# LightwheelAI/street-gaussians-ns

Measured on NVIDIA H100. Metric: rendered frames/sec (fwd+bwd) at 1920x1280, 1M+32x10k Gaussians, higher is better.
Workload: dtype f32

## Files before the change

include/sgn_raster.h:

```cpp
#ifndef SGN_RASTER_H_
#define SGN_RASTER_H_

#include <stddef.h>
#include <stdint.h>

#ifdef __cplusplus
extern "C" {
#endif

#define SGN_ABI_VERSION 2
#define SGN_MAX_FOURIER 8
#define SGN_RECORD_FLOATS 12

typedef enum sgn_status {
    SGN_OK = 0,
    SGN_ERR_INVALID = -1,
    SGN_ERR_CUDA = -2,
    SGN_ERR_WORKSPACE = -3,
    SGN_ERR_OVERFLOW = -4
} sgn_status;


typedef struct sgn_segment {
    int32_t row0;
// ... 53 lines not shown
#define SGN_TUNE_ACC_NO_ROW_SKIP 16
#define SGN_TUNE_FWD_TMA 32

const char* sgn_last_error(void);
int sgn_abi_version(void);
long long sgn_launch_count(void);
size_t sgn_sizeof_segment(void);
size_t sgn_sizeof_segment_grads(void);
size_t sgn_sizeof_camera(void);

int sgn_upload(const void* host, size_t bytes, void* dev, void* stream);

int sgn_project_fwd(const sgn_segment* segs_dev, int nseg, int N, int num_chunks, const sgn_camera* cam,
                    float* records, int32_t* radii, int32_t* num_tiles_hit, uint16_t* tile_bbox,
                    int32_t* tiles_touched, uint32_t* touch_mask, void* stream);

int sgn_project_bwd(const sgn_segment* segs_dev, const sgn_segment_grads* grads_dev, int nseg, int N, int num_chunks,
                    const sgn_camera* cam, const float* records, const int32_t* radii,
                    const float* v_records, void* stream);
int sgn_project_bwd_range(const sgn_segment* segs_dev, const sgn_segment_grads* grads_dev, int nseg, int N, int num_chunks,
                          const sgn_camera* cam, const float* records, const int32_t* radii, const float* v_records,
                          int chunk_begin, int chunk_end, void* stream);

int sgn_l1_project_fwd(int N, const float* means, const float* scales, float glob_scale, const float* quats,
                       const sgn_camera* cam, float* xys, float* depths, int32_t* radii, float* conics,
                       float* compensation, int32_t* num_tiles_hit, float* cov3d, void* stream);
int sgn_l1_project_bwd(int N, const float* means, const float* scales, float glob_scale, const float* quats,
                       const sgn_camera* cam, const int32_t* radii, const float* v_xys, const float* v_depths,
                       const float* v_conics, float* v_means, float* v_scales, float* v_quats, void* stream);
int sgn_l1_sh(int N, int K, int degree, const float* viewdirs, const float* coeffs, const float* v_colors,
              float* colors, float* v_coeffs, void* stream);

int sgn_bin_count(int N, const sgn_camera* cam, const float* records, const int32_t* radii,
                  const uint16_t* tile_bbox, int32_t* tiles_touched, uint32_t* touch_mask, void* stream);
size_t sgn_bin_scan_scratch_bytes(int N);
int sgn_bin_scan(int N, const float* records, const int32_t* radii, const int32_t* tiles_touched,
                 int32_t* order, int32_t* cum, int64_t* total_dev, void* scratch, size_t scratch_bytes, void* stream);
size_t sgn_bin_sort_scratch_bytes(int64_t M);
int sgn_bin_sort(int N, int64_t M, const sgn_camera* cam, const float* records, const int32_t* radii,
                 const uint16_t* tile_bbox, const uint32_t* touch_mask, const int32_t* order, const int32_t* cum,
                 int32_t* sorted_ids , int32_t* tile_bins , void* scratch, size_t scratch_bytes,
                 void* stream);
int sgn_bin_sort_capped(int N, int64_t capacity, const int64_t* total_dev, int32_t* overflow_dev, const sgn_camera* cam,
                        const float* records, const int32_t* radii, const uint16_t* tile_bbox, const uint32_t* touch_mask,
                        const int32_t* order, const int32_t* cum, int32_t* sorted_ids, int32_t* tile_bins, void* scratch,
                        size_t scratch_bytes, void* stream);
int sgn_bin_local_cap(void);
size_t sgn_bin_local_scratch_bytes(int64_t M, int tiles);
int sgn_bin_local_count(int N, const sgn_camera* cam, const float* records, const int32_t* radii, const uint16_t* tile_bbox,
                        const uint32_t* touch_mask, int32_t* tile_count, int32_t* tile_start, int64_t* info_dev, void* scratch,
                        size_t scratch_bytes, void* stream);
int sgn_bin_local_sort(int N, int64_t M, int longest_list, const sgn_camera* cam, const float* records, const int32_t* radii,
// ... 145 lines not shown
```

street-gaussians-ns_b200/_lib.py:

```python
from __future__ import annotations

import ctypes as C
import os

HERE = os.path.dirname(os.path.abspath(__file__))
LIB_PATH = os.path.join(HERE, "libsgn_raster.so")
MAX_FOURIER = 8
RECORD_FLOATS = 12


class SgnError(RuntimeError):
    pass


class Segment(C.Structure):
    _fields_ = [
        ("row0", C.c_int32), ("count", C.c_int32), ("F", C.c_int32), ("cls", C.c_int32),
        ("has_pose", C.c_int32), ("chunk0", C.c_int32),
        ("R", C.c_float * 9), ("t", C.c_float * 3), ("q", C.c_float * 4), ("idft", C.c_float * MAX_FOURIER),
        ("means", C.c_void_p), ("scales", C.c_void_p), ("quats", C.c_void_p),
        ("features_dc", C.c_void_p), ("features_rest", C.c_void_p), ("opacities", C.c_void_p),
    ]


# ... 88 lines not shown
    ]


_lib = None

EXPORTS = [
    "sgn_last_error", "sgn_abi_version", "sgn_launch_count", "sgn_sizeof_segment", "sgn_sizeof_segment_grads", "sgn_sizeof_camera",
    "sgn_upload", "sgn_bin_count", "sgn_project_fwd", "sgn_project_bwd", "sgn_l1_project_fwd", "sgn_l1_project_bwd", "sgn_l1_sh", "sgn_bin_scan_scratch_bytes", "sgn_bin_scan",
    "sgn_bin_sort_scratch_bytes", "sgn_bin_sort", "sgn_bin_class_scratch_bytes", "sgn_bin_class_lists", "sgn_blend_sched_ints",
    "sgn_blend_fwd", "sgn_blend_bwd", "sgn_sizeof_adam_tensor", "sgn_adam_chunk_elems", "sgn_adam_step",
    "sgn_loss_scratch_bytes", "sgn_loss_fwd", "sgn_loss_bwd", "sgn_ssim_workspace_bytes", "sgn_ssim_fwd", "sgn_ssim_bwd",
    "sgn_sizeof_densify_segment", "sgn_densify_stats",
    "sgn_sizeof_refine_config", "sgn_sizeof_refine_tensors", "sgn_refine_decide", "sgn_refine_apply",
    "sgn_bin_local_cap", "sgn_bin_local_scratch_bytes", "sgn_bin_local_count", "sgn_bin_local_sort",
    "sgn_project_bwd_range", "sgn_allreduce_sym", "sgn_blend_extra_fwd", "sgn_blend_extra_bwd",
    "sgn_bin_sort_capped", "sgn_visible_flags", "sgn_visible_union",
]
AR_MAX_SLICES = 48


def load():
    global _lib
    if _lib is not None:
        return _lib
    path = os.environ.get("SGN_RASTER_LIB", LIB_PATH)
    if not os.path.exists(path):
        raise SgnError(
            f"{path} is missing. Build it with `python street-gaussians-ns_b200/build.py` "
            "(or __graft_entry__.build()). There is no CPU fallback for the rasterizer.")
    L = C.CDLL(path)
    vp, i32, i64, sz = C.c_void_p, C.c_int, C.c_int64, C.c_size_t
    L.sgn_last_error.restype = C.c_char_p
    L.sgn_abi_version.restype = C.c_int
    L.sgn_launch_count.restype = C.c_longlong
    for f in ("sgn_sizeof_segment", "sgn_sizeof_segment_grads", "sgn_sizeof_camera"):
        getattr(L, f).restype = sz
    L.sgn_upload.argtypes = [vp, sz, vp, vp]
    L.sgn_project_fwd.argtypes = [vp, i32, i32, i32, C.POINTER(CameraStruct), vp, vp, vp, vp, vp, vp, vp]
    L.sgn_project_bwd.argtypes = [vp, vp, i32, i32, i32, C.POINTER(CameraStruct), vp, vp, vp, vp]
    L.sgn_project_bwd_range.argtypes = [vp, vp, i32, i32, i32, C.POINTER(CameraStruct), vp, vp, vp, i32, i32, vp]
    L.sgn_project_bwd_range.restype = C.c_int
    L.sgn_allreduce_sym.argtypes = [vp, vp, vp, i32, i32, i32, C.POINTER(C.c_int64), C.POINTER(C.c_int64), C.POINTER(C.c_int32),
                                    C.POINTER(C.c_int64), C.POINTER(C.c_int64), vp, C.c_float, i32, vp]
    L.sgn_visible_flags.argtypes = [vp, i64, vp, vp]
    L.sgn_visible_union.argtypes = [vp, i64, i32, i64, vp, vp]
    L.sgn_allreduce_sym.restype = L.sgn_visible_flags.restype = L.sgn_visible_union.restype = C.c_int
    L.sgn_blend_extra_fwd.argtypes = [C.POINTER(CameraStruct), C.POINTER(BlendOpts), vp, vp, vp, vp, vp, vp, i32, vp, vp]
    L.sgn_blend_extra_bwd.argtypes = [C.POINTER(CameraStruct), C.POINTER(BlendOpts), vp, vp, vp, vp, vp, vp, i32, vp, vp, vp, vp]
    L.sgn_blend_extra_fwd.restype = L.sgn_blend_extra_bwd.restype = C.c_int
    fl = C.c_float
    L.sgn_l1_project_fwd.argtypes = [i32, vp, vp, fl, vp, C.POINTER(CameraStruct), vp, vp, vp, vp, vp, vp, vp, vp]
    L.sgn_l1_project_bwd.argtypes = [i32, vp, vp, fl, vp, C.POINTER(CameraStruct), vp, vp, vp, vp, vp, vp, vp, vp]
    L.sgn_l1_sh.argtypes = [i32, i32, i32, vp, vp, vp, vp, vp, vp]
    for f in ("sgn_l1_project_fwd", "sgn_l1_project_bwd", "sgn_l1_sh"):
        getattr(L, f).restype = C.c_int
    L.sgn_bin_scan_scratch_bytes.argtypes = [i32]
    L.sgn_bin_scan_scratch_bytes.restype = sz
    L.sgn_bin_scan.argtypes = [i32, vp, vp, vp, vp, vp, vp, vp, sz, vp]
    L.sgn_bin_count.argtypes = [i32, C.POINTER(CameraStruct), vp, vp, vp, vp, vp, vp]
    L.sgn_bin_count.restype = C.c_int
    L.sgn_bin_sort_scratch_bytes.argtypes = [i64]
    L.sgn_bin_sort_scratch_bytes.restype = sz
    L.sgn_bin_sort.argtypes = [i32, i64, C.POINTER(CameraStruct), vp, vp, vp, vp, vp, vp, vp, vp, vp, sz, vp]
    L.sgn_bin_sort_capped.argtypes = [i32, i64, vp, vp, C.POINTER(CameraStruct), vp, vp, vp, vp, vp, vp, vp, vp, vp, sz, vp]
    L.sgn_bin_sort_capped.restype = C.c_int
    L.sgn_bin_local_cap.restype = C.c_int
    L.sgn_bin_local_scratch_bytes.argtypes = [i64, i32]
    L.sgn_bin_local_scratch_bytes.restype = sz
    L.sgn_bin_local_count.argtypes = [i32, C.POINTER(CameraStruct), vp, vp, vp, vp, vp, vp, vp, vp, sz, vp]
    L.sgn_bin_local_count.restype = C.c_int
    L.sgn_bin_local_sort.argtypes = [i32, i64, i32, C.POINTER(CameraStruct), vp, vp, vp, vp, vp, vp, vp, vp, vp, vp, vp, sz, vp]
    L.sgn_bin_local_sort.restype = C.c_int
    L.sgn_bin_class_scratch_bytes.argtypes = [i32]
# ... 49 lines not shown
```

street-gaussians-ns_b200/csrc/binning.cu:

```cuda
#include <cub/cub.cuh>

#include "sgn_touch.cuh"

static inline size_t align_up(size_t x, size_t a) { return (x + a - 1) / a * a; }

__global__ void __launch_bounds__(256)
count_tiles_kernel(int N, int width, int height, int bw, const float4* __restrict__ records, const int32_t* __restrict__ radii,
                   const ushort4* __restrict__ tile_bbox, int32_t* __restrict__ tiles_touched, uint32_t* __restrict__ touch_mask) {
    const int g = blockIdx.x * blockDim.x + threadIdx.x;
    const bool vis = (g < N) && radii[g] > 0;
    ushort4 bb = make_ushort4(0, 0, 0, 0);
    TouchCtx t = {};
    if (vis) {
        bb = tile_bbox[g];
        t = make_touch_ctx(records[3 * (size_t)g], records[3 * (size_t)g + 1]);
    }
    uint32_t mask;
    const int n = count_touched_tiles(vis, t, bb, width, height, bw, mask);
    if (g < N) { tiles_touched[g] = n; touch_mask[g] = mask; }
}

extern "C" int sgn_bin_count(int N, const sgn_camera* cam, const float* records, const int32_t* radii,
                             const uint16_t* tile_bbox, int32_t* tiles_touched, uint32_t* touch_mask, void* stream) {
    SGN_RANGE("sgn_bin_count");
// ... 20 lines not shown
    }
    keys[g] = key;
    vals[g] = payload;
}

struct PermutedCount {
    const int32_t* order;
    const int32_t* counts;
    __host__ __device__ int32_t operator()(int i) const { return counts[order[i] & 0x7fffffff]; }
};

__global__ void write_total_kernel(const int32_t* __restrict__ cum, int N, int64_t* __restrict__ total) {
    if (threadIdx.x == 0 && blockIdx.x == 0) *total = (N > 0) ? (int64_t)cum[N - 1] : 0;
}

struct ScanLayout {
    size_t keys_in, keys_out, vals_in, temp, temp_bytes, total;
};
static ScanLayout scan_layout(int N) {
    ScanLayout L;
    const size_t n = (size_t)(N > 0 ? N : 1);
    size_t t1 = 0, t2 = 0;
    cub::DeviceRadixSort::SortPairs(nullptr, t1, (const uint32_t*)nullptr, (uint32_t*)nullptr, (const int32_t*)nullptr,
                                    (int32_t*)nullptr, (int)n, 0, 32);
    cub::DeviceScan::InclusiveSum(nullptr, t2, (const int32_t*)nullptr, (int32_t*)nullptr, (int)n);
    L.keys_in = 0;
    L.keys_out = align_up(n * 4, 256);
    L.vals_in = L.keys_out + align_up(n * 4, 256);
    L.temp = L.vals_in + align_up(n * 4, 256);
    L.temp_bytes = t1 > t2 ? t1 : t2;
    L.total = L.temp + align_up(L.temp_bytes, 256) + 256;
    return L;
}

extern "C" size_t sgn_bin_scan_scratch_bytes(int N) { return scan_layout(N).total; }

extern "C" int sgn_bin_scan(int N, const float* records, const int32_t* radii, const int32_t* tiles_touched,
                            int32_t* order , int32_t* cum,
                            int64_t* total_dev, void* scratch, size_t scratch_bytes, void* stream_) {
    SGN_RANGE("sgn_bin_scan");
    cudaStream_t stream = (cudaStream_t)stream_;
    SGN_REQUIRE(records && radii && tiles_touched && order && cum && total_dev && scratch, "sgn_bin_scan: null pointer");
    const ScanLayout L = scan_layout(N);
    if (scratch_bytes < L.total) {
// ... 6 lines not shown
        uint32_t* keys_out = (uint32_t*)(base + L.keys_out);
        int32_t* vals_in = (int32_t*)(base + L.vals_in);
        depth_keys_kernel<<<(N + 255) / 256, 256, 0, stream>>>(N, reinterpret_cast<const float4*>(records), radii, keys_in, vals_in);
        SGN_CHECK_LAUNCH("depth_keys_kernel");
        size_t temp = L.temp_bytes;
        SGN_CHECK_CUDA(cub::DeviceRadixSort::SortPairs(base + L.temp, temp, keys_in, keys_out, vals_in, order, N, 0, 32, stream));
        sgn_count_launch(1);
        cub::CountingInputIterator<int> idx(0);
        cub::TransformInputIterator<int32_t, PermutedCount, cub::CountingInputIterator<int>> it(idx, PermutedCount{order, tiles_touched});
        temp = L.temp_bytes;
        SGN_CHECK_CUDA(cub::DeviceScan::InclusiveSum(base + L.temp, temp, it, cum, N, stream));
        sgn_count_launch(1);
    }
    write_total_kernel<<<1, 32, 0, stream>>>(cum, N, total_dev);
    SGN_CHECK_LAUNCH("write_total_kernel");
    return SGN_OK;
}

#define HUGE_AREA 1024

__device__ __forceinline__ int nth_set_bit(uint32_t m, int k) {
    int pos = 0;
#pragma unroll
    for (int w = 16; w > 0; w >>= 1) {
        const int c = __popc(m & ((1u << w) - 1u));
        if (k >= c) { k -= c; m >>= w; pos += w; }
    }
    return pos;
}

// ... 141 lines not shown
        for (int b = 0; b < r.ar && r.pos < end; b += 32) {
            const int ti = b + lane;
            const int tx = r.x0 + ti % r.wd, ty = r.y0 + ti / r.wd;
            const bool ok = (ti < r.ar) && tile_touched(r.c, tx, ty, width, height, bw);
            const unsigned bal = __ballot_sync(0xffffffffu, ok);
            const int my = r.pos + __popc(bal & lt);
            if (ok && my < end) {
                keys[my] = (uint16_t)(ty * tiles_x + tx);
                vals[my] = r.pl;
            }
            r.pos += __popc(bal);
        }
    }
}

__global__ void __launch_bounds__(256)
bin_edges_kernel(int64_t M, const uint16_t* __restrict__ keys_sorted, int32_t* __restrict__ tile_bins) {
    const int64_t i = (int64_t)blockIdx.x * blockDim.x + threadIdx.x;
    if (i >= M) return;
    const int32_t cur = (int32_t)keys_sorted[i];
    if (i == 0) tile_bins[2 * cur] = 0;
    else {
        const int32_t prev = (int32_t)keys_sorted[i - 1];
        if (prev != cur) {
            tile_bins[2 * prev + 1] = (int32_t)i;
            tile_bins[2 * cur] = (int32_t)i;
        }
    }
    if (i == M - 1) tile_bins[2 * cur + 1] = (int32_t)M;
}

__global__ void __launch_bounds__(256)
bin_edges_capped_kernel(int64_t cap, const int64_t* __restrict__ total, const uint16_t* __restrict__ keys_sorted, int32_t* __restrict__ tile_bins,
                        int32_t* __restrict__ overflow) {
    const int64_t i = (int64_t)blockIdx.x * blockDim.x + threadIdx.x;
    const int64_t M = min(*total, cap);
    if (i == 0 && *total > cap) *overflow = 1;
    if (i >= M) return;
    const int32_t cur = (int32_t)keys_sorted[i];
    if (i == 0) tile_bins[2 * cur] = 0;
    else {
        const int32_t prev = (int32_t)keys_sorted[i - 1];
        if (prev != cur) {
            tile_bins[2 * prev + 1] = (int32_t)i;
            tile_bins[2 * cur] = (int32_t)i;
        }
    }
    if (i == M - 1) tile_bins[2 * cur + 1] = (int32_t)M;
}

struct SortLayout {
    size_t keys_in, keys_out, vals_in, big, temp, temp_bytes, total;
};

static SortLayout sort_layout(int64_t M) {
    SortLayout L;
    const size_t m = (size_t)(M > 0 ? M : 1);
    size_t temp = 0;
    cub::DeviceRadixSort::SortPairs(nullptr, temp, (const uint16_t*)nullptr, (uint16_t*)nullptr, (const int32_t*)nullptr,
                                    (int32_t*)nullptr, (int64_t)m, 0, 16);
    L.keys_in = 0;
    L.keys_out = align_up(L.keys_in + m * 2, 256);
    L.vals_in = align_up(L.keys_out + m * 2, 256);
// ... 38 lines not shown
    SGN_REQUIRE(!total_dev || tile_bits <= 16, "sgn_bin_sort_capped: %d tiles leave no 16-bit key for the padding", tiles);
    emit_keys_kernel<<<(N + 255) / 256, 256, 0, stream>>>(N, tiles_x, reinterpret_cast<const ushort4*>(tile_bbox), touch_mask, order, cum, (int)M,
                                                          total_dev, (uint16_t)((1u << tile_bits) - 1u), keys_in, vals_in, big_ranks,
                                                          big_count);
    SGN_CHECK_LAUNCH("emit_keys_kernel");
    int sms = 0, dev = 0;
    SGN_CHECK_CUDA(cudaGetDevice(&dev));
    SGN_CHECK_CUDA(cudaDeviceGetAttribute(&sms, cudaDevAttrMultiProcessorCount, dev));
    emit_big_kernel<<<4 * sms, EMIT_BIG_THREADS, 0, stream>>>(tiles_x, cam->width, cam->height, bw, reinterpret_cast<const float4*>(records),
                                                 reinterpret_cast<const ushort4*>(tile_bbox), order, cum, (int)M, big_ranks, big_count,
                                                 keys_in, vals_in);
    SGN_CHECK_LAUNCH("emit_big_kernel");
    size_t temp = L.temp_bytes;
    SGN_CHECK_CUDA(cub::DeviceRadixSort::SortPairs(base + L.temp, temp, keys_in, keys_out, vals_in, sorted_ids, M, 0, tile_bits, stream));
    sgn_count_launch(1);
    if (total_dev) {
        bin_edges_capped_kernel<<<(unsigned)((M + 255) / 256), 256, 0, stream>>>(M, total_dev, keys_out, tile_bins, overflow_dev);
        SGN_CHECK_LAUNCH("bin_edges_capped_kernel");
    } else {
        bin_edges_kernel<<<(unsigned)((M + 255) / 256), 256, 0, stream>>>(M, keys_out, tile_bins);
        SGN_CHECK_LAUNCH("bin_edges_kernel");
    }
    return SGN_OK;
}

extern "C" int sgn_bin_sort(int N, int64_t M, const sgn_camera* cam, const float* records, const int32_t* radii,
                            const uint16_t* tile_bbox, const uint32_t* touch_mask, const int32_t* order, const int32_t* cum,
                            int32_t* sorted_ids, int32_t* tile_bins, void* scratch, size_t scratch_bytes, void* stream_) {
    SGN_RANGE("sgn_bin_sort");
    return bin_sort_impl(N, M, nullptr, nullptr, cam, records, radii, tile_bbox, touch_mask, order, cum, sorted_ids, tile_bins, scratch,
                         scratch_bytes, stream_);
}

extern "C" int sgn_bin_sort_capped(int N, int64_t capacity, const int64_t* total_dev, int32_t* overflow_dev, const sgn_camera* cam,
                                   const float* records, const int32_t* radii, const uint16_t* tile_bbox, const uint32_t* touch_mask,
// ... 121 lines not shown
```

street-gaussians-ns_b200/csrc/project.cu:

```cuda
#include <stdarg.h>
#include <stdlib.h>
#include <string.h>

#include "sgn_exact.cuh"
#include "sgn_touch.cuh"

static thread_local char g_err[512] = "";
void sgn_set_error(const char* fmt, ...) {
    va_list ap;
    va_start(ap, fmt);
    vsnprintf(g_err, sizeof(g_err), fmt, ap);
    va_end(ap);
}
#include <atomic>
static std::atomic<long long> g_launches{0};
void sgn_count_launch(int n) { g_launches.fetch_add(n, std::memory_order_relaxed); }
extern "C" long long sgn_launch_count(void) { return g_launches.load(std::memory_order_relaxed); }
extern "C" const char* sgn_last_error(void) { return g_err; }
extern "C" int sgn_abi_version(void) { return SGN_ABI_VERSION; }
extern "C" size_t sgn_sizeof_segment(void) { return sizeof(sgn_segment); }
extern "C" size_t sgn_sizeof_segment_grads(void) { return sizeof(sgn_segment_grads); }
extern "C" size_t sgn_sizeof_camera(void) { return sizeof(sgn_camera); }

extern "C" int sgn_upload(const void* host, size_t bytes, void* dev, void* stream) {
// ... 29 lines not shown
        for (int i = threadIdx.x; i < n; i += blockDim.x) dst[i] = __ldg(src + i);
    }
}
__device__ __forceinline__ void coop_store(float* __restrict__ dst, const float* __restrict__ src, int n) {
    if ((reinterpret_cast<uintptr_t>(dst) & 15u) == 0) {
        const int n4 = n >> 2;
        const float4* s4 = reinterpret_cast<const float4*>(src);
        float4* d4 = reinterpret_cast<float4*>(dst);
        for (int i = threadIdx.x; i < n4; i += blockDim.x) d4[i] = s4[i];
        for (int i = (n4 << 2) + threadIdx.x; i < n; i += blockDim.x) dst[i] = src[i];
    } else {
        for (int i = threadIdx.x; i < n; i += blockDim.x) dst[i] = src[i];
    }
}

__global__ void __launch_bounds__(CH)
project_fwd_direct_kernel(const sgn_segment* __restrict__ segs, int nseg, const sgn_camera cam,
                   float4* __restrict__ records, int32_t* __restrict__ radii, int32_t* __restrict__ num_tiles_hit,
                   ushort4* __restrict__ tile_bbox, int32_t* __restrict__ tiles_touched, uint32_t* __restrict__ touch_mask) {
    extern __shared__ int s_chunk0[];
    for (int i = threadIdx.x; i < nseg; i += blockDim.x) s_chunk0[i] = segs[i].chunk0;
    __syncthreads();
    const int si = find_segment_by_chunk(s_chunk0, nseg, blockIdx.x);
    const sgn_segment& sg = segs[si];
    const int i = (blockIdx.x - sg.chunk0) * CH + threadIdx.x;
    const bool active = i < sg.count;
    const size_t g = (size_t)sg.row0 + i;
    const int K = (cam.sh_degree + 1) * (cam.sh_degree + 1);
    bool vis = false;
    ushort4 bb = make_ushort4(0, 0, 0, 0);
    TouchCtx tc = {};
    if (active) {

    float m[3], ls[3], q[4];
#pragma unroll
    for (int k = 0; k < 3; ++k) { m[k] = __ldg(sg.means + 3 * (size_t)i + k); ls[k] = __ldg(sg.scales + 3 * (size_t)i + k); }
    {
        const float4 qq = __ldg(reinterpret_cast<const float4*>(sg.quats) + i);
        q[0] = qq.x; q[1] = qq.y; q[2] = qq.z; q[3] = qq.w;
    }
    SgnProj st;
    vis = sgn_project_exact(sg, cam, m, ls, q, st);

    float rgb[3] = {0.f, 0.f, 0.f};
    float opac = 0.f;
    int aux = 0;
    if (vis) {
        float c0[3] = {0.f, 0.f, 0.f};
        for (int f = 0; f < sg.F; ++f) {
            const float w = sg.idft[f];
#pragma unroll
            for (int ch = 0; ch < 3; ++ch) c0[ch] += __ldg(sg.features_dc + ((size_t)i * sg.F + f) * 3 + ch) * w;
        }
        if (cam.sh_degree > 0) {
            float d[3] = {st.mw[0] - cam.cam_pos[0], st.mw[1] - cam.cam_pos[1], st.mw[2] - cam.cam_pos[2]};
            const float n = sqrtf(d[0] * d[0] + d[1] * d[1] + d[2] * d[2]);
            d[0] /= n; d[1] /= n; d[2] /= n;
// ... 28 lines not shown
    radii[g] = st.radius;
    num_tiles_hit[g] = vis ? (st.tmax[0] - st.tmin[0]) * (st.tmax[1] - st.tmin[1]) : 0;
    bb = make_ushort4((unsigned short)st.tmin[0], (unsigned short)st.tmin[1],
                      (unsigned short)st.tmax[0], (unsigned short)st.tmax[1]);
    tile_bbox[g] = bb;
    if (vis) tc = make_touch_ctx(make_float4(st.xy[0], st.xy[1], st.conic[0], st.conic[1]), make_float4(st.conic[2], opac, 0.f, 0.f));
    }
    uint32_t mask;
    const int nt = count_touched_tiles(vis, tc, bb, cam.width, cam.height, cam.block_width, mask);
    if (active) {
        tiles_touched[g] = nt;
        touch_mask[g] = mask;
    }
}

__global__ void __launch_bounds__(CH)
project_fwd_staged_kernel(const sgn_segment* __restrict__ segs, int nseg, const sgn_camera cam,
                   float4* __restrict__ records, int32_t* __restrict__ radii, int32_t* __restrict__ num_tiles_hit,
                   ushort4* __restrict__ tile_bbox, int32_t* __restrict__ tiles_touched, uint32_t* __restrict__ touch_mask) {
    extern __shared__ int s_chunk0[];
    __shared__ __align__(16) float s_rest[CH * MAX_REST];
    __shared__ __align__(16) float s_dc[CH * MAX_DC];
    __shared__ __align__(16) float s_means[CH * 3];
    __shared__ __align__(16) float s_scales[CH * 3];
    __shared__ float s_geo[CH][9];
    __shared__ int s_row[CH];
    __shared__ int s_warp_base[CH / 32 + 1];
    for (int i = threadIdx.x; i < nseg; i += blockDim.x) s_chunk0[i] = segs[i].chunk0;
    __syncthreads();
    const int si = find_segment_by_chunk(s_chunk0, nseg, blockIdx.x);
    const sgn_segment& sg = segs[si];
    const int r0 = (blockIdx.x - sg.chunk0) * CH;
    const int rows = min(CH, sg.count - r0);
    const int tid = threadIdx.x, lane = tid & 31, warp = tid >> 5;
// ... 2 lines not shown
    coop_load(s_means, sg.means + 3 * (size_t)r0, rows * 3);
    coop_load(s_scales, sg.scales + 3 * (size_t)r0, rows * 3);
    __syncthreads();

    const bool active = tid < rows;
    const size_t g = (size_t)sg.row0 + r0 + tid;
    const int cls_bit = sg.cls == 1 ? SGN_AUX_OBJECT : 0;
    bool vis = false;
    SgnProj st;
    if (active) {
        const float m[3] = {s_means[3 * tid], s_means[3 * tid + 1], s_means[3 * tid + 2]};
        const float ls[3] = {s_scales[3 * tid], s_scales[3 * tid + 1], s_scales[3 * tid + 2]};
        const float4 qq = __ldg(reinterpret_cast<const float4*>(sg.quats) + r0 + tid);
        const float q[4] = {qq.x, qq.y, qq.z, qq.w};
        vis = sgn_project_exact(sg, cam, m, ls, q, st);
        radii[g] = st.radius;
        num_tiles_hit[g] = vis ? (st.tmax[0] - st.tmin[0]) * (st.tmax[1] - st.tmin[1]) : 0;
        tile_bbox[g] = make_ushort4((unsigned short)st.tmin[0], (unsigned short)st.tmin[1],
                                    (unsigned short)st.tmax[0], (unsigned short)st.tmax[1]);
        float4* rec = records + 3 * g;
        rec[0] = make_float4(st.xy[0], st.xy[1], st.conic[0], st.conic[1]);
        if (!vis) {
            rec[1] = make_float4(st.conic[2], 0.f, 0.f, 0.f);
            rec[2] = make_float4(0.f, 0.f, __int_as_float(cls_bit), 0.f);
            tiles_touched[g] = 0;
            touch_mask[g] = 0u;
        }
    }
    const unsigned bal = __ballot_sync(0xffffffffu, vis);
    if (lane == 0) s_warp_base[warp + 1] = __popc(bal);
// ... 88 lines not shown
        float4* rec = records + 3 * gb;
        rec[1] = make_float4(ge[4], opac, rgb[0], rgb[1]);
        rec[2] = make_float4(rgb[2], ge[5], __int_as_float(aux), 0.f);
        bb = tile_bbox[gb];
        tc = make_touch_ctx(make_float4(ge[0], ge[1], ge[2], ge[3]), make_float4(ge[4], opac, 0.f, 0.f));
    }
    if ((warp << 5) >= nvis) return;
    uint32_t mask;
    const int nt = count_touched_tiles(mine, tc, bb, cam.width, cam.height, cam.block_width, mask);
    if (mine) {
        tiles_touched[gb] = nt;
        touch_mask[gb] = mask;
    }
}

extern "C" int sgn_project_fwd(const sgn_segment* segs_dev, int nseg, int N, int num_chunks, const sgn_camera* cam,
                               float* records, int32_t* radii, int32_t* num_tiles_hit, uint16_t* tile_bbox,
                               int32_t* tiles_touched, uint32_t* touch_mask, void* stream) {
    SGN_RANGE("sgn_project_fwd");
    SGN_REQUIRE(segs_dev && cam && records && radii && num_tiles_hit && tile_bbox && tiles_touched && touch_mask,
                "sgn_project_fwd: null pointer");
    SGN_REQUIRE(nseg >= 1 && nseg <= SGN_MAX_SEGMENTS, "sgn_project_fwd: nseg=%d out of range [1,%d]", nseg, SGN_MAX_SEGMENTS);
    SGN_REQUIRE(N >= 0 && num_chunks >= 0, "sgn_project_fwd: negative size");
    SGN_REQUIRE(cam->block_width >= 2 && cam->block_width <= 16, "block_width must be between 2 and 16 (got %d)", cam->block_width);
    SGN_REQUIRE(cam->sh_degree >= 0 && cam->sh_degree <= 3 && cam->sh_degree_to_use >= 0 && cam->sh_degree_to_use <= cam->sh_degree,
                "sh_degree must be in [0,3] and sh_degree_to_use <= sh_degree");
    SGN_REQUIRE((cam->width + cam->block_width - 1) / cam->block_width < 65536 && (cam->height + cam->block_width - 1) / cam->block_width < 65536,
                "image too large for 16-bit tile coordinates");
    SGN_REQUIRE(sgn_aligned16(records), "records must be 16-byte aligned");
    if (N == 0 || num_chunks == 0) return SGN_OK;
    const char* staged_env = getenv("SGN_PROJECT_STAGED");
    if (staged_env && staged_env[0] == '1')
        project_fwd_staged_kernel<<<num_chunks, CH, nseg * sizeof(int), (cudaStream_t)stream>>>(
            segs_dev, nseg, *cam, reinterpret_cast<float4*>(records), radii, num_tiles_hit,
            reinterpret_cast<ushort4*>(tile_bbox), tiles_touched, touch_mask);
    else
        project_fwd_direct_kernel<<<num_chunks, CH, nseg * sizeof(int), (cudaStream_t)stream>>>(
            segs_dev, nseg, *cam, reinterpret_cast<float4*>(records), radii, num_tiles_hit,
            reinterpret_cast<ushort4*>(tile_bbox), tiles_touched, touch_mask);
    SGN_CHECK_LAUNCH("project_fwd_kernel");
    return SGN_OK;
}

__device__ __forceinline__ void sgn_project_vjp(const sgn_camera& cam, const SgnProj& st, const float v_xy[2], float v_depth,
                                                const float v_conic[3], float vmw[3], float vs[3], float vqr[4]) {
    const float* W = cam.viewmat;
    const float fx = cam.fx, fy = cam.fy;
    float vpv[3];
    {
        const float rw = 1.f / (st.pv[2] + 1e-6f);
        const float vx = fx * v_xy[0], vy = fy * v_xy[1];
        vpv[0] = vx * rw;
        vpv[1] = vy * rw;
        vpv[2] = -(vx * st.pv[0] + vy * st.pv[1]) * rw * rw + v_depth;
    }
    float vA, vB, vC;
// ... 347 lines not shown
```

street-gaussians-ns_b200/raster.py:

```python
from __future__ import annotations

import ctypes as C
import os
from dataclasses import dataclass
from typing import Dict, List, Optional

import numpy as np
import torch

from . import _lib
from . import scene as scene_mod
from .scene import PARAM_NAMES, Camera, Frame


@dataclass
class RenderSettings:
    sh_degree: int = 3
    sh_degree_to_use: Optional[int] = None
    block_width: int = 16
    clip_thresh: float = 0.01
    alpha_clamp_fwd: float = 0.999
    alpha_clamp_bwd: float = 0.99
    class_streams: bool = True
    training: bool = True
# ... 156 lines not shown
        if slot is not None and upload:
            slot["table"] = self


def _grads_table(arena: torch.Tensor, static: dict, device) -> torch.Tensor:
    off = static.get("grad_offsets")
    if off is None:
        flat = np.array([x for ss in static["sizes"] for x in ss], np.uint64)
        off = static["grad_offsets"] = (np.concatenate([[0], np.cumsum(flat)[:-1]]) * 4).astype(np.uint64)
    tab = (np.uint64(arena.data_ptr()) + off).view(np.uint8)
    return torch.from_numpy(tab).to(device, non_blocking=True)


class Projected:

    def __init__(self, records, radii, tiles_hit, bbox, tiles_touched, touch_mask):
        self.records, self.radii, self.tiles_hit, self.bbox = records, radii, tiles_hit, bbox
        self.tiles_touched, self.touch_mask = tiles_touched, touch_mask

    def __iter__(self):
        return iter((self.records, self.radii, self.tiles_hit, self.bbox))


def project_fwd(table: SegmentTable, cs: _lib.CameraStruct, device) -> Projected:
    L = _lib.load()
    N = table.N
    records = torch.empty(N, _lib.RECORD_FLOATS, device=device, dtype=torch.float32)
    ints = torch.empty(4, max(N, 1), device=device, dtype=torch.int32)
    bbox = torch.empty(N, 4, device=device, dtype=torch.int16)
    with _timed("project_fwd"):
        _lib.check(L.sgn_project_fwd(_ptr(table.dev), table.nseg, N, table.num_chunks, C.byref(cs), _ptr(records), _ptr(ints[0]),
                                     _ptr(ints[1]), _ptr(bbox), _ptr(ints[2]), _ptr(ints[3]), _stream()), "sgn_project_fwd")
    return Projected(records, ints[0][:N], ints[1][:N], bbox, ints[2][:N], ints[3][:N])


BIN_LOCAL = os.environ.get("SGN_BIN_LOCAL", "0") == "1"


def _bin_local(cs: _lib.CameraStruct, records, radii, proj: Projected):
    L = _lib.load()
    device = records.device
    N = records.shape[0]
    bw = cs.block_width
    tiles = ((cs.width + bw - 1) // bw) * ((cs.height + bw - 1) // bw)
    counts = torch.empty(2, tiles, device=device, dtype=torch.int32)
    info = torch.empty(2, device=device, dtype=torch.int64)
    sb = L.sgn_bin_local_scratch_bytes(0, tiles)
    scratch = torch.empty(sb, device=device, dtype=torch.uint8)
# ... 110 lines not shown
        if res is not None:
            return res
    if proj is not None:
        bbox, touched, mask = proj.bbox, proj.tiles_touched, proj.touch_mask
    else:
        touched = torch.empty(max(N, 1), device=device, dtype=torch.int32)
        mask = torch.empty(max(N, 1), device=device, dtype=torch.int32)
        with _timed("bin_count"):
            _lib.check(L.sgn_bin_count(N, C.byref(cs), _ptr(records), _ptr(radii), _ptr(bbox), _ptr(touched), _ptr(mask),
                                       _stream()), "sgn_bin_count")
    oc = torch.empty(2, max(N, 1), device=device, dtype=torch.int32)
    total = torch.empty(1, device=device, dtype=torch.int64)
    sb = L.sgn_bin_scan_scratch_bytes(N)
    scratch = torch.empty(sb, device=device, dtype=torch.uint8)
    with _timed("bin_scan"):
        _lib.check(L.sgn_bin_scan(N, _ptr(records), _ptr(radii), _ptr(touched), _ptr(oc[0]), _ptr(oc[1]), _ptr(total),
                                  _ptr(scratch), sb, _stream()), "sgn_bin_scan")
    bw = cs.block_width
    tiles = ((cs.width + bw - 1) // bw) * ((cs.height + bw - 1) // bw)
    tile_bins = torch.empty(tiles, 2, device=device, dtype=torch.int32)
    if use_async and N > 0 and tiles < 65536:
        st = _async_state(device)
        _async_poll(st)
        if st["max_m"] > 0:
            cap = int((int(st["max_m"] * ASYNC_HEADROOM) + ASYNC_GRANULE - 1) // ASYNC_GRANULE * ASYNC_GRANULE)
            pin = st["pinned"][st["slot"] % len(st["pinned"])]
            st["slot"] += 1
            pin.copy_(total, non_blocking=True)
            ev = torch.cuda.Event()
            ev.record()
            lazy = LazyCount(ev, pin, cap, total)
            st["pending"].append(lazy)
# ... 354 lines not shown
```

Before: 440.2.

## Emit depth sort keys in projection and fuse gather-scan with decoupled lookback

The projection kernel now also writes per-Gaussian depth keys and indexed values, so binning can radix-sort them directly instead of building keys in a separate pass. A new single-pass decoupled-lookback scan kernel gathers tiles_touched in sorted order and computes the cumulative sum plus the total in one launch. The bin-edges kernel is also merged into a single grid-stride version with vectorized key loads. This removes a key-construction pass and extra launches, at the cost of extra global writes in projection and a more complex scan with inter-block spinning.

```diff
diff --git a/include/sgn_raster.h b/include/sgn_raster.h
--- a/include/sgn_raster.h
+++ b/include/sgn_raster.h
@@ -91,6 +91,9 @@
 int sgn_project_fwd(const sgn_segment* segs_dev, int nseg, int N, int num_chunks, const sgn_camera* cam,
                     float* records, int32_t* radii, int32_t* num_tiles_hit, uint16_t* tile_bbox,
                     int32_t* tiles_touched, uint32_t* touch_mask, void* stream);
+int sgn_project_fwd_keys(const sgn_segment* segs_dev, int nseg, int N, int num_chunks, const sgn_camera* cam,
+                         float* records, int32_t* radii, int32_t* num_tiles_hit, uint16_t* tile_bbox,
+                         int32_t* tiles_touched, uint32_t* touch_mask, uint32_t* depth_keys, int32_t* depth_vals, void* stream);
 
 int sgn_project_bwd(const sgn_segment* segs_dev, const sgn_segment_grads* grads_dev, int nseg, int N, int num_chunks,
                     const sgn_camera* cam, const float* records, const int32_t* radii,
@@ -113,6 +116,8 @@
 size_t sgn_bin_scan_scratch_bytes(int N);
 int sgn_bin_scan(int N, const float* records, const int32_t* radii, const int32_t* tiles_touched,
                  int32_t* order, int32_t* cum, int64_t* total_dev, void* scratch, size_t scratch_bytes, void* stream);
+int sgn_bin_scan_keys(int N, const uint32_t* depth_keys, const int32_t* depth_vals, const int32_t* tiles_touched,
+                      int32_t* order, int32_t* cum, int64_t* total_dev, void* scratch, size_t scratch_bytes, void* stream);
 size_t sgn_bin_sort_scratch_bytes(int64_t M);
 int sgn_bin_sort(int N, int64_t M, const sgn_camera* cam, const float* records, const int32_t* radii,
                  const uint16_t* tile_bbox, const uint32_t* touch_mask, const int32_t* order, const int32_t* cum,
diff --git a/street-gaussians-ns_b200/_lib.py b/street-gaussians-ns_b200/_lib.py
--- a/street-gaussians-ns_b200/_lib.py
+++ b/street-gaussians-ns_b200/_lib.py
@@ -126,7 +126,7 @@
     "sgn_sizeof_refine_config", "sgn_sizeof_refine_tensors", "sgn_refine_decide", "sgn_refine_apply",
     "sgn_bin_local_cap", "sgn_bin_local_scratch_bytes", "sgn_bin_local_count", "sgn_bin_local_sort",
     "sgn_project_bwd_range", "sgn_allreduce_sym", "sgn_blend_extra_fwd", "sgn_blend_extra_bwd",
-    "sgn_bin_sort_capped", "sgn_visible_flags", "sgn_visible_union",
+    "sgn_bin_sort_capped", "sgn_visible_flags", "sgn_visible_union", "sgn_project_fwd_keys", "sgn_bin_scan_keys",
 ]
 AR_MAX_SLICES = 48
 
@@ -149,6 +149,8 @@
         getattr(L, f).restype = sz
     L.sgn_upload.argtypes = [vp, sz, vp, vp]
     L.sgn_project_fwd.argtypes = [vp, i32, i32, i32, C.POINTER(CameraStruct), vp, vp, vp, vp, vp, vp, vp]
+    L.sgn_project_fwd_keys.argtypes = [vp, i32, i32, i32, C.POINTER(CameraStruct), vp, vp, vp, vp, vp, vp, vp, vp, vp]
+    L.sgn_project_fwd_keys.restype = C.c_int
     L.sgn_project_bwd.argtypes = [vp, vp, i32, i32, i32, C.POINTER(CameraStruct), vp, vp, vp, vp]
     L.sgn_project_bwd_range.argtypes = [vp, vp, i32, i32, i32, C.POINTER(CameraStruct), vp, vp, vp, i32, i32, vp]
     L.sgn_project_bwd_range.restype = C.c_int
@@ -169,6 +171,8 @@
     L.sgn_bin_scan_scratch_bytes.argtypes = [i32]
     L.sgn_bin_scan_scratch_bytes.restype = sz
     L.sgn_bin_scan.argtypes = [i32, vp, vp, vp, vp, vp, vp, vp, sz, vp]
+    L.sgn_bin_scan_keys.argtypes = [i32, vp, vp, vp, vp, vp, vp, vp, sz, vp]
+    L.sgn_bin_scan_keys.restype = C.c_int
     L.sgn_bin_count.argtypes = [i32, C.POINTER(CameraStruct), vp, vp, vp, vp, vp, vp]
     L.sgn_bin_count.restype = C.c_int
     L.sgn_bin_sort_scratch_bytes.argtypes = [i64]
diff --git a/street-gaussians-ns_b200/csrc/binning.cu b/street-gaussians-ns_b200/csrc/binning.cu
--- a/street-gaussians-ns_b200/csrc/binning.cu
+++ b/street-gaussians-ns_b200/csrc/binning.cu
@@ -58,8 +58,69 @@
     if (threadIdx.x == 0 && blockIdx.x == 0) *total = (N > 0) ? (int64_t)cum[N - 1] : 0;
 }
 
+#define SCAN_THREADS 256
+#define SCAN_ITEMS 8
+#define SCAN_TILE (SCAN_THREADS * SCAN_ITEMS)
+
+__global__ void __launch_bounds__(SCAN_THREADS)
+depth_scan_kernel(int N, int tiles, const int32_t* __restrict__ order, const int32_t* __restrict__ counts, int32_t* __restrict__ cum,
+                  int64_t* __restrict__ total, unsigned long long* __restrict__ state, unsigned int* __restrict__ ticket) {
+    typedef cub::BlockScan<int, SCAN_THREADS> BlockScan;
+    __shared__ typename BlockScan::TempStorage tmp;
+    __shared__ int s_tile, s_prefix;
+    if (threadIdx.x == 0) s_tile = (int)atomicAdd(ticket, 1u);
+    __syncthreads();
+    const int t = s_tile;
+    const int base = t * SCAN_TILE + threadIdx.x * SCAN_ITEMS;
+    int v[SCAN_ITEMS];
+    int sum = 0;
+#pragma unroll
+    for (int j = 0; j < SCAN_ITEMS; ++j) {
+        const int r = base + j;
+        v[j] = r < N ? counts[order[r] & 0x7fffffff] : 0;
+        sum += v[j];
+    }
+    int excl, agg;
+    BlockScan(tmp).ExclusiveSum(sum, excl, agg);
+    if (threadIdx.x < 32) {
+        const int lane = threadIdx.x;
+        volatile unsigned long long* vs = state;
+        int prefix = 0;
+        if (t == 0) {
+            if (lane == 0) vs[0] = (2ull << 62) | (unsigned)agg;
+        } else {
+            if (lane == 0) vs[t] = (1ull << 62) | (unsigned)agg;
+            for (int w = t - 1; ; w -= 32) {
+                unsigned long long s;
+                do {
+                    s = w - lane >= 0 ? vs[w - lane] : (2ull << 62);
+                } while (__any_sync(0xffffffffu, (s >> 62) == 0));
+                const unsigned inc = __ballot_sync(0xffffffffu, (s >> 62) == 2);
+                const int stop = inc ? __ffs(inc) - 1 : 31;
+                int p = lane <= stop ? (int)(s & 0x7fffffffu) : 0;
+#pragma unroll
+                for (int d = 16; d > 0; d >>= 1) p += __shfl_xor_sync(0xffffffffu, p, d);
+                prefix += p;
+                if (inc) break;
+            }
+            if (lane == 0) vs[t] = (2ull << 62) | (unsigned)(prefix + agg);
+        }
+        if (lane == 0) {
+            s_prefix = prefix;
+            if (t == tiles - 1) *total = (int64_t)(prefix + agg);
+        }
+    }
+    __syncthreads();
+    int run = s_prefix + excl;
+#pragma unroll
+    for (int j = 0; j < SCAN_ITEMS; ++j) {
+        run += v[j];
+        if (base + j < N) cum[base + j] = run;
+    }
+}
+
 struct ScanLayout {
-    size_t keys_in, keys_out, vals_in, temp, temp_bytes, total;
+    size_t keys_in, keys_out, vals_in, state, state_bytes, temp, temp_bytes, total;
 };
 static ScanLayout scan_layout(int N) {
     ScanLayout L;
@@ -71,7 +132,9 @@
     L.keys_in = 0;
     L.keys_out = align_up(n * 4, 256);
     L.vals_in = L.keys_out + align_up(n * 4, 256);
-    L.temp = L.vals_in + align_up(n * 4, 256);
+    L.state = L.vals_in + align_up(n * 4, 256);
+    L.state_bytes = align_up(sizeof(unsigned long long) * ((n + SCAN_TILE - 1) / SCAN_TILE), 256) + 256;
+    L.temp = L.state + L.state_bytes;
     L.temp_bytes = t1 > t2 ? t1 : t2;
     L.total = L.temp + align_up(L.temp_bytes, 256) + 256;
     return L;
@@ -108,6 +171,34 @@
     }
     write_total_kernel<<<1, 32, 0, stream>>>(cum, N, total_dev);
     SGN_CHECK_LAUNCH("write_total_kernel");
+    return SGN_OK;
+}
+
+extern "C" int sgn_bin_scan_keys(int N, const uint32_t* depth_keys, const int32_t* depth_vals, const int32_t* tiles_touched,
+                                 int32_t* order, int32_t* cum, int64_t* total_dev, void* scratch, size_t scratch_bytes, void* stream_) {
+    SGN_RANGE("sgn_bin_scan");
+    cudaStream_t stream = (cudaStream_t)stream_;
+    SGN_REQUIRE(depth_keys && depth_vals && tiles_touched && order && cum && total_dev && scratch, "sgn_bin_scan_keys: null pointer");
+    const ScanLayout L = scan_layout(N);
+    if (scratch_bytes < L.total) {
+        sgn_set_error("sgn_bin_scan_keys: scratch too small (%zu < %zu)", scratch_bytes, L.total);
+        return SGN_ERR_WORKSPACE;
+    }
+    if (N == 0) {
+        SGN_CHECK_CUDA(cudaMemsetAsync(total_dev, 0, sizeof(int64_t), stream));
+        return SGN_OK;
+    }
+    char* base = (char*)scratch;
+    size_t temp = L.temp_bytes;
+    SGN_CHECK_CUDA(cub::DeviceRadixSort::SortPairs(base + L.temp, temp, depth_keys, (uint32_t*)(base + L.keys_out), depth_vals, order, N,
+                                                   0, 32, stream));
+    sgn_count_launch(1);
+    SGN_CHECK_CUDA(cudaMemsetAsync(base + L.state, 0, L.state_bytes, stream));
+    const int tiles = (N + SCAN_TILE - 1) / SCAN_TILE;
+    depth_scan_kernel<<<tiles, SCAN_THREADS, 0, stream>>>(N, tiles, order, tiles_touched, cum, total_dev,
+                                                          (unsigned long long*)(base + L.state),
+                                                          (unsigned int*)(base + L.state + L.state_bytes - 256));
+    SGN_CHECK_LAUNCH("depth_scan_kernel");
     return SGN_OK;
 }
 
@@ -279,39 +370,38 @@
     }
 }
 
+#define EDGE_KEYS 8
+
 __global__ void __launch_bounds__(256)
-bin_edges_kernel(int64_t M, const uint16_t* __restrict__ keys_sorted, int32_t* __restrict__ tile_bins) {
-    const int64_t i = (int64_t)blockIdx.x * blockDim.x + threadIdx.x;
-    if (i >= M) return;
-    const int32_t cur = (int32_t)keys_sorted[i];
-    if (i == 0) tile_bins[2 * cur] = 0;
-    else {
-        const int32_t prev = (int32_t)keys_sorted[i - 1];
-        if (prev != cur) {
-            tile_bins[2 * prev + 1] = (int32_t)i;
-            tile_bins[2 * cur] = (int32_t)i;
-        }
-    }
-    if (i == M - 1) tile_bins[2 * cur + 1] = (int32_t)M;
-}
-
-__global__ void __launch_bounds__(256)
-bin_edges_capped_kernel(int64_t cap, const int64_t* __restrict__ total, const uint16_t* __restrict__ keys_sorted, int32_t* __restrict__ tile_bins,
-                        int32_t* __restrict__ overflow) {
-    const int64_t i = (int64_t)blockIdx.x * blockDim.x + threadIdx.x;
-    const int64_t M = min(*total, cap);
-    if (i == 0 && *total > cap) *overflow = 1;
-    if (i >= M) return;
-    const int32_t cur = (int32_t)keys_sorted[i];
-    if (i == 0) tile_bins[2 * cur] = 0;
-    else {
-        const int32_t prev = (int32_t)keys_sorted[i - 1];
-        if (prev != cur) {
-            tile_bins[2 * prev + 1] = (int32_t)i;
-            tile_bins[2 * cur] = (int32_t)i;
-        }
-    }
-    if (i == M - 1) tile_bins[2 * cur + 1] = (int32_t)M;
+bin_edges_kernel(int64_t cap, const int64_t* __restrict__ total, const uint16_t* __restrict__ keys_sorted, int32_t* __restrict__ tile_bins,
+                 int32_t* __restrict__ overflow) {
+    const int64_t M = total ? min(*total, cap) : cap;
+    if (total && blockIdx.x == 0 && threadIdx.x == 0 && *total > cap) *overflow = 1;
+    const int64_t stride = (int64_t)gridDim.x * blockDim.x * EDGE_KEYS;
+    for (int64_t i0 = ((int64_t)blockIdx.x * blockDim.x + threadIdx.x) * EDGE_KEYS; i0 < M; i0 += stride) {
+        uint16_t k[EDGE_KEYS];
+        if (i0 + EDGE_KEYS <= M) {
+            const uint4 v = *reinterpret_cast<const uint4*>(keys_sorted + i0);
+            *reinterpret_cast<uint4*>(k) = v;
+        } else {
+#pragma unroll
+            for (int j = 0; j < EDGE_KEYS; ++j) k[j] = i0 + j < M ? keys_sorted[i0 + j] : 0;
+        }
+        int32_t prev = i0 > 0 ? (int32_t)keys_sorted[i0 - 1] : -1;
+#pragma unroll
+        for (int j = 0; j < EDGE_KEYS; ++j) {
+            const int64_t i = i0 + j;
+            if (i >= M) break;
+            const int32_t cur = (int32_t)k[j];
+            if (i == 0) tile_bins[2 * cur] = 0;
+            else if (prev != cur) {
+                tile_bins[2 * prev + 1] = (int32_t)i;
+                tile_bins[2 * cur] = (int32_t)i;
+            }
+            if (i == M - 1) tile_bins[2 * cur + 1] = (int32_t)M;
+            prev = cur;
+        }
+    }
 }
 
 struct SortLayout {
@@ -380,11 +470,11 @@
     size_t temp = L.temp_bytes;
     SGN_CHECK_CUDA(cub::DeviceRadixSort::SortPairs(base + L.temp, temp, keys_in, keys_out, vals_in, sorted_ids, M, 0, tile_bits, stream));
     sgn_count_launch(1);
-    if (total_dev) {
-        bin_edges_capped_kernel<<<(unsigned)((M + 255) / 256), 256, 0, stream>>>(M, total_dev, keys_out, tile_bins, overflow_dev);
-        SGN_CHECK_LAUNCH("bin_edges_capped_kernel");
-    } else {
-        bin_edges_kernel<<<(unsigned)((M + 255) / 256), 256, 0, stream>>>(M, keys_out, tile_bins);
+    {
+        const int64_t groups = (M + EDGE_KEYS - 1) / EDGE_KEYS;
+        const int64_t want = (groups + 255) / 256;
+        const int blocks = (int)(want < (int64_t)16 * sms ? want : (int64_t)16 * sms);
+        bin_edges_kernel<<<blocks, 256, 0, stream>>>(M, total_dev, keys_out, tile_bins, overflow_dev);
         SGN_CHECK_LAUNCH("bin_edges_kernel");
     }
     return SGN_OK;
diff --git a/street-gaussians-ns_b200/csrc/project.cu b/street-gaussians-ns_b200/csrc/project.cu
--- a/street-gaussians-ns_b200/csrc/project.cu
+++ b/street-gaussians-ns_b200/csrc/project.cu
@@ -67,10 +67,22 @@
     }
 }
 
+struct DepthKeysOut {
+    uint32_t* keys;
+    int32_t* vals;
+};
+
+__device__ __forceinline__ void write_depth_key(const DepthKeysOut& dk, bool vis, size_t g, float depth, int cls) {
+    dk.keys[g] = vis ? (uint32_t)__float_as_int(depth) : 0xffffffffu;
+    dk.vals[g] = (int32_t)g | (vis && cls == 1 ? (int32_t)0x80000000 : 0);
+}
+
+template <bool KEYS>
 __global__ void __launch_bounds__(CH)
 project_fwd_direct_kernel(const sgn_segment* __restrict__ segs, int nseg, const sgn_camera cam,
                    float4* __restrict__ records, int32_t* __restrict__ radii, int32_t* __restrict__ num_tiles_hit,
-                   ushort4* __restrict__ tile_bbox, int32_t* __restrict__ tiles_touched, uint32_t* __restrict__ touch_mask) {
+                   ushort4* __restrict__ tile_bbox, int32_t* __restrict__ tiles_touched, uint32_t* __restrict__ touch_mask,
+                   const DepthKeysOut dk) {
     extern __shared__ int s_chunk0[];
     for (int i = threadIdx.x; i < nseg; i += blockDim.x) s_chunk0[i] = segs[i].chunk0;
     __syncthreads();
@@ -94,6 +106,7 @@
     }
     SgnProj st;
     vis = sgn_project_exact(sg, cam, m, ls, q, st);
+    if (KEYS) write_depth_key(dk, vis, g, st.pv[2], sg.cls);
 
     float rgb[3] = {0.f, 0.f, 0.f};
     float opac = 0.f;
@@ -152,10 +165,12 @@
     }
 }
 
+template <bool KEYS>
 __global__ void __launch_bounds__(CH)
 project_fwd_staged_kernel(const sgn_segment* __restrict__ segs, int nseg, const sgn_camera cam,
                    float4* __restrict__ records, int32_t* __restrict__ radii, int32_t* __restrict__ num_tiles_hit,
-                   ushort4* __restrict__ tile_bbox, int32_t* __restrict__ tiles_touched, uint32_t* __restrict__ touch_mask) {
+                   ushort4* __restrict__ tile_bbox, int32_t* __restrict__ tiles_touched, uint32_t* __restrict__ touch_mask,
+                   const DepthKeysOut dk) {
     extern __shared__ int s_chunk0[];
     __shared__ __align__(16) float s_rest[CH * MAX_REST];
     __shared__ __align__(16) float s_dc[CH * MAX_DC];
@@ -188,6 +203,7 @@
         const float4 qq = __ldg(reinterpret_cast<const float4*>(sg.quats) + r0 + tid);
         const float q[4] = {qq.x, qq.y, qq.z, qq.w};
         vis = sgn_project_exact(sg, cam, m, ls, q, st);
+        if (KEYS) write_depth_key(dk, vis, g, st.pv[2], sg.cls);
         radii[g] = st.radius;
         num_tiles_hit[g] = vis ? (st.tmax[0] - st.tmin[0]) * (st.tmax[1] - st.tmin[1]) : 0;
         tile_bbox[g] = make_ushort4((unsigned short)st.tmin[0], (unsigned short)st.tmin[1],
@@ -306,10 +322,9 @@
     }
 }
 
-extern "C" int sgn_project_fwd(const sgn_segment* segs_dev, int nseg, int N, int num_chunks, const sgn_camera* cam,
-                               float* records, int32_t* radii, int32_t* num_tiles_hit, uint16_t* tile_bbox,
-                               int32_t* tiles_touched, uint32_t* touch_mask, void* stream) {
-    SGN_RANGE("sgn_project_fwd");
+static int project_fwd_impl(const sgn_segment* segs_dev, int nseg, int N, int num_chunks, const sgn_camera* cam, float* records,
+                            int32_t* radii, int32_t* num_tiles_hit, uint16_t* tile_bbox, int32_t* tiles_touched, uint32_t* touch_mask,
+                            const DepthKeysOut* dk, cudaStream_t stream) {
     SGN_REQUIRE(segs_dev && cam && records && radii && num_tiles_hit && tile_bbox && tiles_touched && touch_mask,
                 "sgn_project_fwd: null pointer");
     SGN_REQUIRE(nseg >= 1 && nseg <= SGN_MAX_SEGMENTS, "sgn_project_fwd: nseg=%d out of range [1,%d]", nseg, SGN_MAX_SEGMENTS);
@@ -322,16 +337,32 @@
     SGN_REQUIRE(sgn_aligned16(records), "records must be 16-byte aligned");
     if (N == 0 || num_chunks == 0) return SGN_OK;
     const char* staged_env = getenv("SGN_PROJECT_STAGED");
-    if (staged_env && staged_env[0] == '1')
-        project_fwd_staged_kernel<<<num_chunks, CH, nseg * sizeof(int), (cudaStream_t)stream>>>(
-            segs_dev, nseg, *cam, reinterpret_cast<float4*>(records), radii, num_tiles_hit,
-            reinterpret_cast<ushort4*>(tile_bbox), tiles_touched, touch_mask);
-    else
-        project_fwd_direct_kernel<<<num_chunks, CH, nseg * sizeof(int), (cudaStream_t)stream>>>(
-            segs_dev, nseg, *cam, reinterpret_cast<float4*>(records), radii, num_tiles_hit,
-            reinterpret_cast<ushort4*>(tile_bbox), tiles_touched, touch_mask);
+    const bool staged = staged_env && staged_env[0] == '1';
+    const DepthKeysOut none = {};
+    auto kernel = staged ? (dk ? project_fwd_staged_kernel<true> : project_fwd_staged_kernel<false>)
+                         : (dk ? project_fwd_direct_kernel<true> : project_fwd_direct_kernel<false>);
+    kernel<<<num_chunks, CH, nseg * sizeof(int), stream>>>(segs_dev, nseg, *cam, reinterpret_cast<float4*>(records), radii, num_tiles_hit,
+                                                           reinterpret_cast<ushort4*>(tile_bbox), tiles_touched, touch_mask, dk ? *dk : none);
     SGN_CHECK_LAUNCH("project_fwd_kernel");
     return SGN_OK;
+}
+
+extern "C" int sgn_project_fwd(const sgn_segment* segs_dev, int nseg, int N, int num_chunks, const sgn_camera* cam,
+                               float* records, int32_t* radii, int32_t* num_tiles_hit, uint16_t* tile_bbox,
+                               int32_t* tiles_touched, uint32_t* touch_mask, void* stream) {
+    SGN_RANGE("sgn_project_fwd");
+    return project_fwd_impl(segs_dev, nseg, N, num_chunks, cam, records, radii, num_tiles_hit, tile_bbox, tiles_touched, touch_mask,
+                            nullptr, (cudaStream_t)stream);
+}
+
+extern "C" int sgn_project_fwd_keys(const sgn_segment* segs_dev, int nseg, int N, int num_chunks, const sgn_camera* cam,
+                                    float* records, int32_t* radii, int32_t* num_tiles_hit, uint16_t* tile_bbox,
+                                    int32_t* tiles_touched, uint32_t* touch_mask, uint32_t* depth_keys, int32_t* depth_vals, void* stream) {
+    SGN_RANGE("sgn_project_fwd");
+    SGN_REQUIRE(depth_keys && depth_vals, "sgn_project_fwd_keys: null pointer");
+    const DepthKeysOut dk = {depth_keys, depth_vals};
+    return project_fwd_impl(segs_dev, nseg, N, num_chunks, cam, records, radii, num_tiles_hit, tile_bbox, tiles_touched, touch_mask, &dk,
+                            (cudaStream_t)stream);
 }
 
 __device__ __forceinline__ void sgn_project_vjp(const sgn_camera& cam, const SgnProj& st, const float v_xy[2], float v_depth,
diff --git a/street-gaussians-ns_b200/raster.py b/street-gaussians-ns_b200/raster.py
--- a/street-gaussians-ns_b200/raster.py
+++ b/street-gaussians-ns_b200/raster.py
@@ -194,9 +194,10 @@
 
 class Projected:
 
-    def __init__(self, records, radii, tiles_hit, bbox, tiles_touched, touch_mask):
+    def __init__(self, records, radii, tiles_hit, bbox, tiles_touched, touch_mask, depth_keys=None):
         self.records, self.radii, self.tiles_hit, self.bbox = records, radii, tiles_hit, bbox
         self.tiles_touched, self.touch_mask = tiles_touched, touch_mask
+        self.depth_keys = depth_keys
 
     def __iter__(self):
         return iter((self.records, self.radii, self.tiles_hit, self.bbox))
@@ -206,12 +207,13 @@
     L = _lib.load()
     N = table.N
     records = torch.empty(N, _lib.RECORD_FLOATS, device=device, dtype=torch.float32)
-    ints = torch.empty(4, max(N, 1), device=device, dtype=torch.int32)
+    ints = torch.empty(6, max(N, 1), device=device, dtype=torch.int32)
     bbox = torch.empty(N, 4, device=device, dtype=torch.int16)
     with _timed("project_fwd"):
-        _lib.check(L.sgn_project_fwd(_ptr(table.dev), table.nseg, N, table.num_chunks, C.byref(cs), _ptr(records), _ptr(ints[0]),
-                                     _ptr(ints[1]), _ptr(bbox), _ptr(ints[2]), _ptr(ints[3]), _stream()), "sgn_project_fwd")
-    return Projected(records, ints[0][:N], ints[1][:N], bbox, ints[2][:N], ints[3][:N])
+        _lib.check(L.sgn_project_fwd_keys(_ptr(table.dev), table.nseg, N, table.num_chunks, C.byref(cs), _ptr(records), _ptr(ints[0]),
+                                          _ptr(ints[1]), _ptr(bbox), _ptr(ints[2]), _ptr(ints[3]), _ptr(ints[4]), _ptr(ints[5]), _stream()),
+                   "sgn_project_fwd_keys")
+    return Projected(records, ints[0][:N], ints[1][:N], bbox, ints[2][:N], ints[3][:N], depth_keys=(ints[4][:N], ints[5][:N]))
 
 
 BIN_LOCAL = os.environ.get("SGN_BIN_LOCAL", "0") == "1"
@@ -352,8 +354,13 @@
     sb = L.sgn_bin_scan_scratch_bytes(N)
     scratch = torch.empty(sb, device=device, dtype=torch.uint8)
     with _timed("bin_scan"):
-        _lib.check(L.sgn_bin_scan(N, _ptr(records), _ptr(radii), _ptr(touched), _ptr(oc[0]), _ptr(oc[1]), _ptr(total),
-                                  _ptr(scratch), sb, _stream()), "sgn_bin_scan")
+        if proj is not None and proj.depth_keys is not None:
+            keys, vals = proj.depth_keys
+            _lib.check(L.sgn_bin_scan_keys(N, _ptr(keys), _ptr(vals), _ptr(touched), _ptr(oc[0]), _ptr(oc[1]), _ptr(total),
+                                           _ptr(scratch), sb, _stream()), "sgn_bin_scan_keys")
+        else:
+            _lib.check(L.sgn_bin_scan(N, _ptr(records), _ptr(radii), _ptr(touched), _ptr(oc[0]), _ptr(oc[1]), _ptr(total),
+                                      _ptr(scratch), sb, _stream()), "sgn_bin_scan")
     bw = cs.block_width
     tiles = ((cs.width + bw - 1) // bw) * ((cs.height + bw - 1) // bw)
     tile_bins = torch.empty(tiles, 2, device=device, dtype=torch.int32)
```

Result: no change. 442.6 (median of 6 runs) (+0.5%).
